# yoraish/mmd

Measured on AMD Instinct MI355X. Metric: guided trajectories/sec (H=64, 100 denoise steps), 32-robot Empty map, higher is better.
Workload: dtype f32 (f16x2 split on the fp16 MFMA pipe: every fp32 product as 3 fp16 MFMAs, fp32 accumulate)

## Files before the change

### mmd_amd/csrc/guide.hip

```cpp
#include <hip/hip_runtime.h>

#include <atomic>
#include <cmath>

#include "../../include/mmd_amd.h"
#include "../../include/mmd_amd_debug.h"
#include "bins_dev.h"
#include "common.h"
#include "guide_dev.h"

namespace mmd {

__device__ __forceinline__ float clip_scale(float gx, float gy, float gz, float gw, float max_norm) {
  const float ax = gx + 1e-6f, ay = gy + 1e-6f, az = gz + 1e-6f, aw = gw + 1e-6f;
  const float n2 = ax * ax + ay * ay + az * az + aw * aw;
  return fminf(max_norm * __builtin_amdgcn_rsqf(n2), 1.f);
}

__device__ __forceinline__ bool clip_grad(const GuideDev& g, float& gx, float& gy, float& gz, float& gw) {
  if (g.clip_rule == 0) {
    const float sc = clip_scale(gx, gy, gz, gw, g.max_norm);
    gx = sc * gx; gy = sc * gy; gz = sc * gz; gw = sc * gw;
    return sc < 1.f;
  } else if (g.clip_rule == 1) {
    const float m = g.max_value;
    const bool on = fabsf(gx) > m || fabsf(gy) > m || fabsf(gz) > m || fabsf(gw) > m;
    gx = fminf(fmaxf(gx, -m), m); gy = fminf(fmaxf(gy, -m), m); gz = fminf(fmaxf(gz, -m), m); gw = fminf(fmaxf(gw, -m), m);
    return on;
  }
  return false;
}
__device__ __forceinline__ bool clip_grad(const GuideDev& g, float& gx, float& gy) {
  float z = 0.f, w = 0.f;
  return clip_grad(g, gx, gy, z, w);
}

__device__ __forceinline__ float lane_prev(float v) {
  return __builtin_bit_cast(float, __builtin_amdgcn_update_dpp(0, __builtin_bit_cast(int, v), 0x138, 0xf, 0xf, true));
}
__device__ __forceinline__ float lane_next(float v) {
  return __builtin_bit_cast(float, __builtin_amdgcn_update_dpp(0, __builtin_bit_cast(int, v), 0x130, 0xf, 0xf, true));
}

constexpr int LDS_SLOTS_SMALL = 40;
constexpr int LDS_SLOTS_MAX = 144;

__device__ __forceinline__ float rsq_pos(float d2) { return __builtin_amdgcn_rsqf(fmaxf(d2, 1e-30f)); }

typedef float f32x2g __attribute__((ext_vector_type(2)));
struct Acc4 { f32x2g a0, a1, a2, a3; };
__device__ __forceinline__ Acc4 acc4_zero() {
  const f32x2g z = {0.f, 0.f};
  return Acc4{z, z, z, z};
}
__device__ __forceinline__ f32x2g acc4_total(const Acc4& r) {
  return f32x2g{(r.a0.x + r.a1.x) + (r.a2.x + r.a3.x), (r.a0.y + r.a1.y) + (r.a2.y + r.a3.y)};
}
__device__ __forceinline__ f32x2g cons_term(f32x2g a, f32x2g p, f32x2g q, float r2) {
  const float dx = p.x - q.x, dy = p.y - q.y;
  const float d2 = __builtin_fmaf(dx, dx, dy * dy);
  const float m = (d2 > r2) ? 0.f : rsq_pos(d2);
  return f32x2g{__builtin_fmaf(-dx, m, a.x), __builtin_fmaf(-dy, m, a.y)};
}
template <bool COMPACT> struct ConsTab;
template <> struct ConsTab<false> {
  const float4* tab;
  float r2;
  __device__ __forceinline__ f32x2g add(f32x2g a, f32x2g p, int slot, int t) const {
    const float4 c = tab[slot * H + t];
    return cons_term(a, p, f32x2g{c.x, c.y}, c.w);
  }
};
template <> struct ConsTab<true> {
  const float2* tab;
  float r2;
  __device__ __forceinline__ f32x2g add(f32x2g a, f32x2g p, int slot, int t) const {
    const float2 c = tab[slot * H + t];
    return cons_term(a, p, f32x2g{c.x, c.y}, r2);
  }
};
template <class TAB>
__device__ __forceinline__ void cons_accumulate4(Acc4& acc, const TAB& tab, int first, int n, int rel, int t, f32x2g p) {
  auto one = [&](int k, int slot) {
    if (k == 0) acc.a0 = tab.add(acc.a0, p, slot, t);
    else if (k == 1) acc.a1 = tab.add(acc.a1, p, slot, t);
    else if (k == 2) acc.a2 = tab.add(acc.a2, p, slot, t);
    else acc.a3 = tab.add(acc.a3, p, slot, t);
  };
  int i = 0;
  for (; i < n && ((rel + i) & 3); ++i) one((rel + i) & 3, first + i);
#pragma unroll 2
  for (; i + 3 < n; i += 4) {
    acc.a0 = tab.add(acc.a0, p, first + i, t);
    acc.a1 = tab.add(acc.a1, p, first + i + 1, t);
    acc.a2 = tab.add(acc.a2, p, first + i + 2, t);
    acc.a3 = tab.add(acc.a3, p, first + i + 3, t);
  }
  for (int k = 0; i < n; ++i, ++k) one(k, first + i);
}
template <class TAB>
__device__ __forceinline__ f32x2g cons_accumulate1(f32x2g a, const TAB& tab, int first, int n, int rel, int k, int t, f32x2g p) {
#pragma unroll 4
  for (int j = (k - rel) & 3; j < n; j += 4) a = tab.add(a, p, first + j, t);
  return a;
}

struct GroupMeta {
  static constexpr bool kOneGroup = false;
  int s0[2], s1[2];
  float w[2];
  int grp0, n;
  __device__ __forceinline__ void load(const GuideDev& g, int g0, int g1) {
    grp0 = g0;
    n = min(g1 - g0, 2);
#pragma unroll
    for (int k = 0; k < 2; ++k) {
      s0[k] = s1[k] = 0;
      w[k] = 0.f;
      if (k < n) {
        s0[k] = __builtin_amdgcn_readfirstlane(g.grp_slot_off[g0 + k]);
        s1[k] = __builtin_amdgcn_readfirstlane(g.grp_slot_off[g0 + k + 1]);
        w[k] = __builtin_bit_cast(float, __builtin_amdgcn_readfirstlane(__builtin_bit_cast(int, g.grp_weight[g0 + k])));
      }
    }
  }
  __device__ __forceinline__ void bounds(const GuideDev& g, int grp, int& a, int& b) const {
    const int k = grp - grp0;
    if (k == 0 && n > 0) { a = s0[0]; b = s1[0]; }
    else if (k == 1 && n > 1) { a = s0[1]; b = s1[1]; }
    else { a = __builtin_amdgcn_readfirstlane(g.grp_slot_off[grp]); b = __builtin_amdgcn_readfirstlane(g.grp_slot_off[grp + 1]); }
  }
  __device__ __forceinline__ float weight(const GuideDev& g, int grp) const {
    const int k = grp - grp0;
    return (k == 0 && n > 0) ? w[0] : (k == 1 && n > 1) ? w[1] : g.grp_weight[grp];
  }
};

template <bool DUMP = false, class GROUPSUM, class GROUPW>
__device__ __forceinline__ float4 guide_grad(const GuideDev& g, float4 xn, int t, const float4* __restrict__ grid,
                                             int grp0, int grp1, GROUPSUM group_sum, GROUPW group_weight, unsigned int* tr = nullptr) {
  unsigned int flags = 0;
  float xu[4];
  const float xv[4] = {xn.x, xn.y, xn.z, xn.w};
#pragma unroll
  for (int d = 0; d < 4; ++d) {
    float v = fminf(fmaxf(xv[d], -1.f), 1.f);
    if constexpr (DUMP) flags |= (fabsf(xv[d]) > 1.f ? 1u : 0u) << (16 + d);
    v = (v + 1.f) / 2.f;
    xu[d] = v * g.nscale[d] + g.nmin[d];
  }
  const float px = xu[0], py = xu[1], vx = xu[2], vy = xu[3];
  const bool interior = t > 0 && t < H - 1;

  int ix = (int)floorf((px - g.lo[0]) / g.dim[0] * (float)g.nx);
  int iy = (int)floorf((py - g.lo[1]) / g.dim[1] * (float)g.ny);
  ix = min(max(ix, 0), g.nx - 1);
  iy = min(max(iy, 0), g.ny - 1);
  const float4 cell0 = g.n_grids > 0 ? grid[(size_t)ix * g.ny + iy] : make_float4(1e30f, 0.f, 0.f, 0.f);

  float wsx, wsy;
  {
    const float d0 = px - g.ws_min[0], d1 = py - g.ws_min[1], d2 = g.ws_max[0] - px, d3 = g.ws_max[1] - py;
    float best = fmaxf(g.margin - d0, 0.f), gx = -1.f, gy = 0.f;
    float v = fmaxf(g.margin - d1, 0.f);
    if (v > best) { best = v; gx = 0.f; gy = -1.f; }
    v = fmaxf(g.margin - d2, 0.f);
    if (v > best) { best = v; gx = 1.f; gy = 0.f; }
    v = fmaxf(g.margin - d3, 0.f);
    if (v > best) { best = v; gx = 0.f; gy = 1.f; }
    if (!(best > 0.f)) { gx = 0.f; gy = 0.f; }
    if constexpr (DUMP) {
      const unsigned arg = gx < 0.f ? 0u : gy < 0.f ? 1u : gx > 0.f ? 2u : 3u;
      if (best > 0.f) flags |= 1u << 4 | arg << 5;
    }
    const bool clipped = clip_grad(g, gx, gy);
    if constexpr (DUMP) flags |= (clipped ? 1u : 0u) << 9;
    wsx = g.w_coll * gx; wsy = g.w_coll * gy;
  }
  float gpx, gpy, gpz, gpw;
  {
    const float npx = lane_next(px), npy = lane_next(py), nvx = lane_next(vx), nvy = lane_next(vy);
    float wpx = 0.f, wpy = 0.f, wvx = 0.f, wvy = 0.f;
    if (t < H - 1) {
      const float epx = npx - (px + g.dt * vx), epy = npy - (py + g.dt * vy);
      const float evx = nvx - vx, evy = nvy - vy;
      wpx = 2.f * (g.m1 * epx + g.m2 * evx);
      wpy = 2.f * (g.m1 * epy + g.m2 * evy);
      wvx = 2.f * (g.m2 * epx + g.m3 * evx);
      wvy = 2.f * (g.m2 * epy + g.m3 * evy);
    }
    const float lpx = lane_prev(wpx), lpy = lane_prev(wpy), lvx = lane_prev(wvx), lvy = lane_prev(wvy);
    float gx = lpx - wpx, gy = lpy - wpy;
    float gz = lvx - (g.dt * wpx + wvx), gw = lvy - (g.dt * wpy + wvy);
    const bool clipped = clip_grad(g, gx, gy, gz, gw);
    if constexpr (DUMP) flags |= (clipped ? 1u : 0u) << 10;
    gpx = g.w_smooth * gx; gpy = g.w_smooth * gy;
    gpz = g.w_smooth * gz; gpw = g.w_smooth * gw;
  }
  float cx = 0.f, cy = 0.f;
  for (int grp = grp0; grp < grp1; ++grp) {
    const f32x2g gs = group_sum(grp, f32x2g{px, py});
    float gx = gs.x, gy = gs.y;
    const bool clipped = clip_grad(g, gx, gy);
    if constexpr (DUMP) {
      const int k = grp - grp0, s0 = g.grp_slot_off[grp], s1 = g.grp_slot_off[grp + 1];
      unsigned long long mask = 0;
      unsigned int n_act = 0;
      for (int sl = s0; sl < s1; ++sl) {
        const float4 c = g.cons[(size_t)sl * H + t];
        const float dx = px - c.x, dy = py - c.y;
        const float d2 = __builtin_fmaf(dx, dx, dy * dy);
        if (!(d2 > c.w)) {
          ++n_act;
          if (sl - s0 < 64) mask |= 1ull << (sl - s0);
        }
      }
      if (k < 4) {
        tr[2 + 2 * k] = (unsigned int)mask;
        tr[3 + 2 * k] = (unsigned int)(mask >> 32);
        flags |= (clipped ? 1u : 0u) << (11 + k);
      }
      tr[10] += n_act;
    }
    const float w = group_weight(grp);
    cx += w * gx; cy += w * gy;
  }
  float ox, oy;
  {
    float best = fmaxf(g.margin - cell0.x, 0.f), gx = 0.f, gy = 0.f;
    unsigned win = 0;
    if (best > 0.f) { gx = -cell0.y; gy = -cell0.z; }
    for (int k = 1; k < g.n_grids; ++k) {
      const float4 c = grid[((size_t)k * g.nx + ix) * g.ny + iy];
      const float v = fmaxf(g.margin - c.x, 0.f);
      if (v > best) { best = v; gx = -c.y; gy = -c.z; win = (unsigned)k; }
    }
    if (g.n_xs + g.n_xb > 0) {
      float ex, ey;
      const float v = fmaxf(g.margin - extra_sdf(g.xs, g.n_xs, g.xb, g.n_xb, px, py, ex, ey), 0.f);
      if (v > best) { best = v; gx = -ex; gy = -ey; win = 7u; }
    }
    const bool clipped = clip_grad(g, gx, gy);
    if constexpr (DUMP) {
      if (best > 0.f) flags |= 1u | (win & 7u) << 1;
      flags |= (clipped ? 1u : 0u) << 8;
    }
    ox = g.w_coll * gx; oy = g.w_coll * gy;
  }
  if constexpr (DUMP) {
    tr[0] = (unsigned int)(ix * g.ny + iy);
    tr[1] = flags | (unsigned int)min(grp1 - grp0, 15) << 20;
  }
  float tx = ((ox + wsx) + gpx) + cx, ty = ((oy + wsy) + gpy) + cy;
  float tz = gpz, tw = gpw;
  if (!interior) { tx = ty = tz = tw = 0.f; }
  return make_float4(-tx, -ty, -tz, -tw);
}


template <bool COMPACT, int NT>
__device__ __forceinline__ void stage_cons(const GuideDev& g, int robot, int lds_slots, float4* lds_cons, int& lds_slot0, int& lds_n) {
  lds_slot0 = __builtin_amdgcn_readfirstlane(g.grp_slot_off[g.robot_grp_off[robot]]);
  lds_n = min(__builtin_amdgcn_readfirstlane(g.grp_slot_off[g.robot_grp_off[robot + 1]]) - lds_slot0, lds_slots);
  const float4* src = g.cons + (size_t)lds_slot0 * H;
  if constexpr (COMPACT) {
    float2* dst = reinterpret_cast<float2*>(lds_cons);
    for (int i = threadIdx.x; i < lds_n * H; i += NT) {
      const float4 c = src[i];
      dst[i] = c.z < 0.f ? make_float2(1e30f, 1e30f) : make_float2(c.x, c.y);
    }
  } else {
    for (int i = threadIdx.x; i < lds_n * H; i += NT) lds_cons[i] = src[i];
  }
}

template <bool COMPACT, class ACC>
__device__ __forceinline__ void group_slots(const GuideDev& g, const GroupMeta& gm, int grp, const float4* lds_cons, int lds_slot0, int lds_n,
                                            ACC acc) {
  int s0, s1;
  gm.bounds(g, grp, s0, s1);
  const int l0 = min(max(s0 - lds_slot0, 0), lds_n), l1 = min(max(s1 - lds_slot0, 0), lds_n);
  if (l1 > l0) {
    if constexpr (COMPACT) acc(ConsTab<true>{reinterpret_cast<const float2*>(lds_cons), g.uniform_r2}, l0, l1 - l0, lds_slot0 + l0 - s0);
    else acc(ConsTab<false>{lds_cons, 0.f}, l0, l1 - l0, lds_slot0 + l0 - s0);
  }
  const int g0 = lds_n > 0 ? max(s0, lds_slot0 + lds_n) : s0;
  if (s1 > g0) acc(ConsTab<false>{g.cons, 0.f}, g0, s1 - g0, g0 - s0);
}

__device__ __forceinline__ float4 model_update(StepDev s, float4 v, const float4* eps, size_t idx) {
  if (s.do_model)
    v = s.ddim == 2 ? ddim_update_x0(v, eps[idx], s.a_t, s.b_t, s.c1, s.c2)
        : s.ddim ? ddim_update(v, eps[idx], s.a_t, s.b_t, s.c1, s.c2) : ddpm_posterior_mean(v, eps[idx], s.a_t, s.b_t, s.c1, s.c2);
  return v;
}

template <bool DUMP, class META = GroupMeta, class GROUPSUM>
__device__ __forceinline__ void guide_iterations(const GuideDev& g, const StepDev& s, int robot, int t, size_t idx, float4& v, bool is_hard,
                                                 float4 hv, bool store, GROUPSUM group_sum) {
  const int map = g.robot_map ? g.robot_map[robot] : 0;
  const float4* grid = g.grids + (size_t)map * g.n_grids * g.nx * g.ny;
  int grp0 = 0, grp1 = 0;
  if constexpr (META::kOneGroup) {
    grp1 = 1;
  } else if (g.robot_grp_off) {
    grp0 = __builtin_amdgcn_readfirstlane(g.robot_grp_off[robot]);
    grp1 = __builtin_amdgcn_readfirstlane(g.robot_grp_off[robot + 1]);
  }
  META gm;
  if constexpr (META::kOneGroup) gm.w = group_sum.weight;
  gm.load(g, grp0, grp1);
  for (int it = 0; it < s.n_guide_steps; ++it) {
    unsigned int* tr = nullptr;
    if constexpr (DUMP) {
      tr = s.trace + ((size_t)it * s.guide_chain_stride + idx) * MMD_TRACE_WORDS;
      for (int w = 0; w < MMD_TRACE_WORDS; ++w) tr[w] = 0u;
    }
    const float4 gr = guide_grad<DUMP>(g, v, t, grid, grp0, grp1, [&](int grp, f32x2g p) { return group_sum(gm, grp, p); },
                                       [&](int grp) { return gm.weight(g, grp); }, tr);
    v.x = __builtin_fmaf(s.grad_scale, gr.x, v.x); v.y = __builtin_fmaf(s.grad_scale, gr.y, v.y);
    v.z = __builtin_fmaf(s.grad_scale, gr.z, v.z); v.w = __builtin_fmaf(s.grad_scale, gr.w, v.w);
    if (is_hard) v = hv;
    if (s.guide_chain && store) s.guide_chain[(size_t)it * s.guide_chain_stride + idx] = v;
  }
}

__device__ __forceinline__ void step_finish(const StepDev& s, float4* x, const float4* noise, float4* chain, size_t idx, int robot,
                                            int samples_per_robot, float4& v, bool is_hard, const float4& hv) {
  if (s.do_noise) v = add_step_noise(v, noise ? noise[idx] : traj_normal4(s.seed, s.robot_seeds, s.draw, s.traj_base, idx, robot, samples_per_robot), s.sigma, s.noise_std_extra);
  if (is_hard) v = hv;
  x[idx] = v;
  if (chain) chain[idx] = v;
}

template <int WPB, bool COMPACT, bool DUMP = false>
__global__ __launch_bounds__(WPB * 64) void ddpm_guide_kernel(GuideDev g, StepDev s, int lds_slots, float4* __restrict__ x,
                                                         const float4* __restrict__ eps,
                                                         const float4* __restrict__ noise, float4* __restrict__ chain,
                                                         const float4* __restrict__ hard,
                                                         int samples_per_robot) {
  extern __shared__ __attribute__((aligned(16))) float4 lds_cons[];
  const int t = threadIdx.x & 63;
  const int traj_b = s.traj0 + blockIdx.x * WPB;
  const int traj = traj_b + (threadIdx.x >> 6);
  const bool valid = traj < s.traj_end;

  int lds_slot0 = 0, lds_n = 0;
  if (s.do_guide && g.robot_grp_off) {
    const int rb0 = traj_b / samples_per_robot;
    const int rb1 = min(traj_b + WPB - 1, s.traj_end - 1) / samples_per_robot;
    if (rb0 == rb1) stage_cons<COMPACT, WPB * 64>(g, rb0, lds_slots, lds_cons, lds_slot0, lds_n);
  }
  __syncthreads();
  if (!valid) return;

  const int robot = traj / samples_per_robot;
  const size_t idx = (size_t)traj * H + t;
  float4 v = model_update(s, x[idx], eps, idx);
  float4 hv = v;
  const bool is_hard = hard_row(s.hard_rows, s.n_hard, hard, robot, t, hv);
  if constexpr (DUMP) {
    if (s.mu_out) s.mu_out[idx] = v;
  }
  if (s.do_guide)
    guide_iterations<DUMP>(g, s, robot, t, idx, v, is_hard, hv, true, [&](const GroupMeta& gm, int grp, f32x2g p) {
      Acc4 acc = acc4_zero();
      group_slots<COMPACT>(g, gm, grp, lds_cons, lds_slot0, lds_n,
                           [&](const auto& tab, int first, int n, int rel) { cons_accumulate4(acc, tab, first, n, rel, t, p); });
      return acc4_total(acc);
    });
  step_finish(s, x, noise, chain, idx, robot, samples_per_robot, v, is_hard, hv);
}

constexpr int COOP_XCH_BYTES = 2 * 4 * H * 8;
template <bool COMPACT>
__global__ __launch_bounds__(256) void ddpm_guide_coop_kernel(GuideDev g, StepDev s, int lds_slots, float4* __restrict__ x,
                                                              const float4* __restrict__ eps, const float4* __restrict__ noise,
                                                              float4* __restrict__ chain, const float4* __restrict__ hard,
                                                              int samples_per_robot) {
  extern __shared__ __attribute__((aligned(16))) float4 lds_cons[];
  const int t = threadIdx.x & 63, wave = __builtin_amdgcn_readfirstlane(threadIdx.x >> 6);
  const int traj = s.traj0 + blockIdx.x;
  const int robot = traj / samples_per_robot;
  float2* const xch = reinterpret_cast<float2*>(reinterpret_cast<char*>(lds_cons) + (size_t)lds_slots * H * (COMPACT ? 8 : 16));
  int lds_slot0 = 0, lds_n = 0;
  if (s.do_guide && g.robot_grp_off) stage_cons<COMPACT, 256>(g, robot, lds_slots, lds_cons, lds_slot0, lds_n);
  __syncthreads();
  const size_t idx = (size_t)traj * H + t;
  float4 v = model_update(s, x[idx], eps, idx);
  float4 hv = v;
  const bool is_hard = hard_row(s.hard_rows, s.n_hard, hard, robot, t, hv);
  if (s.do_guide) {
    int parity = 0;
    guide_iterations<false>(g, s, robot, t, idx, v, is_hard, hv, wave == 0, [&](const GroupMeta& gm, int grp, f32x2g p) {
      f32x2g a = {0.f, 0.f};
      group_slots<COMPACT>(g, gm, grp, lds_cons, lds_slot0, lds_n,
                           [&](const auto& tab, int first, int n, int rel) { a = cons_accumulate1(a, tab, first, n, rel, wave, t, p); });
      float2* const slot = xch + parity * 4 * H;
      slot[wave * H + t] = make_float2(a.x, a.y);
      __syncthreads();
      parity ^= 1;
      const float2 q0 = slot[t], q1 = slot[H + t], q2 = slot[2 * H + t], q3 = slot[3 * H + t];
      return acc4_total(Acc4{f32x2g{q0.x, q0.y}, f32x2g{q1.x, q1.y}, f32x2g{q2.x, q2.y}, f32x2g{q3.x, q3.y}});
    });
  }
  if (wave != 0) return;
  step_finish(s, x, noise, chain, idx, robot, samples_per_robot, v, is_hard, hv);
}


struct OneGroup {
  static constexpr bool kOneGroup = true;
  float w;
  __device__ __forceinline__ void load(const GuideDev&, int, int) {}
  __device__ __forceinline__ float weight(const GuideDev&, int) const { return w; }
};

struct BinnedSum {
  const mmd_cons_bins& b;
  int t, self;
  float r2, weight;
  __device__ __forceinline__ f32x2g operator()(const OneGroup&, int, f32x2g p) const {
    const CellList cl = own_cell_list(b, t, p.x, p.y);
    const float4 none = make_float4(0.f, 0.f, __builtin_bit_cast(float, self), 0.f);
    Acc4 acc = acc4_zero();
    const int last = max(cl.e1 - 1, 0);
    for (int e = cl.e0; __builtin_amdgcn_ballot_w64(e < cl.e1) != 0; e += 4) {
      float4 c[4];
#pragma unroll
      for (int j = 0; j < 4; ++j) {
        const float4 l = cl.ent[min(e + j, last)];
        c[j] = e + j < cl.e1 ? l : none;
      }
#pragma unroll
      for (int j = 0; j < 4; ++j) {
        const int id = __builtin_bit_cast(int, c[j].z);
        const int k = (id - (id > self ? 1 : 0)) & 3;
        f32x2g a = k == 0 ? acc.a0 : k == 1 ? acc.a1 : k == 2 ? acc.a2 : acc.a3;
        a = cons_term(a, p, f32x2g{c[j].x, c[j].y}, id != self ? r2 : -1.f);
        acc.a0 = k == 0 ? a : acc.a0;
        acc.a1 = k == 1 ? a : acc.a1;
        acc.a2 = k == 2 ? a : acc.a2;
        acc.a3 = k == 3 ? a : acc.a3;
      }
    }
    return acc4_total(acc);
  }
};

__global__ __launch_bounds__(256) void ddpm_guide_binned_kernel(GuideDev g, StepDev s, mmd_cons_bins b, float4* __restrict__ x,
                                                                const float4* __restrict__ eps, const float4* __restrict__ noise,
                                                                float4* __restrict__ chain, const float4* __restrict__ hard,
                                                                int samples_per_robot) {
  const int t = threadIdx.x & 63;
  const int traj = s.traj0 + blockIdx.x * 4 + (threadIdx.x >> 6);
  if (traj >= s.traj_end) return;
  const int robot = traj / samples_per_robot;
  const size_t idx = (size_t)traj * H + t;
  float4 v = model_update(s, x[idx], eps, idx);
  float4 hv = v;
  const bool is_hard = hard_row(s.hard_rows, s.n_hard, hard, robot, t, hv);
  if (s.do_guide)
    guide_iterations<false, OneGroup>(g, s, robot, t, idx, v, is_hard, hv, true,
                                      BinnedSum{b, t, b.robot0 + robot, b.radius * fabsf(b.radius), b.weight});
  step_finish(s, x, noise, chain, idx, robot, samples_per_robot, v, is_hard, hv);
}

__global__ void init_kernel(float4* __restrict__ x, float4* __restrict__ chain, const float4* __restrict__ hard,
                            unsigned long long hard_rows, int draw_noise, unsigned long long seed,
                            const unsigned long long* __restrict__ robot_seeds, long long traj_base, int n_traj, int samples_per_robot) {
  const size_t idx = (size_t)blockIdx.x * blockDim.x + threadIdx.x;
  if (idx >= (size_t)n_traj * H) return;
  const int t = idx % H;
  const int robot = (idx / H) / samples_per_robot;
  float4 v = draw_noise ? traj_normal4(seed, robot_seeds, 0xFFFFFFFFu, traj_base, idx, robot, samples_per_robot) : x[idx];
  float4 hv;
  if (hard_row(hard_rows, __popcll(hard_rows), hard, robot, t, hv)) v = hv;
  x[idx] = v;
  if (chain) chain[idx] = v;
}

__global__ void q_sample_kernel(float4* __restrict__ x, const float4* __restrict__ x0, const float4* __restrict__ noise,
                                float a, float b, unsigned long long seed, unsigned int draw, long long traj_base,
                                size_t n_pts) {
  const size_t idx = (size_t)blockIdx.x * blockDim.x + threadIdx.x;
  if (idx >= n_pts) return;
  const float4 z = noise ? noise[idx] : normal4(seed, draw, (unsigned long long)traj_base * H + idx);
  const float4 s = x0[idx];
  x[idx] = make_float4(a * s.x + b * z.x, a * s.y + b * z.y, a * s.z + b * z.z, a * s.w + b * z.w);
}

__global__ void cross_condition_kernel(float4* __restrict__ x1, float4* __restrict__ x2, float4* __restrict__ c1,
                                       float4* __restrict__ c2, int ind1, int ind2, float4 rel, float4 bnd,
                                       const float4* __restrict__ by_robot, int spr, int n_traj) {
  const int b = blockIdx.x * blockDim.x + threadIdx.x;
  if (b >= n_traj) return;
  if (by_robot) {
    rel = by_robot[(size_t)(b / spr) * 2];
    bnd = by_robot[(size_t)(b / spr) * 2 + 1];
  }
  const float4 v2 = x2[(size_t)b * H + ind2];
  float4 v1;
  v1.x = fminf(v2.x + rel.x, bnd.x); v1.y = fminf(v2.y + rel.y, bnd.y);
  v1.z = fminf(v2.z + rel.z, bnd.z); v1.w = fminf(v2.w + rel.w, bnd.w);
  x1[(size_t)b * H + ind1] = v1;
  float4 w;
  w.x = fmaxf(v1.x - rel.x, -bnd.x); w.y = fmaxf(v1.y - rel.y, -bnd.y);
  w.z = fmaxf(v1.z - rel.z, -bnd.z); w.w = fmaxf(v1.w - rel.w, -bnd.w);
  x2[(size_t)b * H + ind2] = w;
  if (c1) c1[(size_t)b * H + ind1] = v1;
  if (c2) c2[(size_t)b * H + ind2] = w;
}

int fill_guide(const mmd_guide_desc* d, GuideDev& g) {
  MMD_REQUIRE(d->n_grids == 0 || (d->sdf_grids_dev && d->grid_nx >= 1 && d->grid_ny >= 1), "guide: SDF grid missing");
  if (d->cons_bins) {
    MMD_REQUIRE(!d->cons_ell_dev, "guide: cons_bins together with an ELL table (cons_ell_dev) is not supported");
    if (int rc = check_cons_bins(d->cons_bins)) return rc;
  }
  for (int k = 0; k < 4; ++k) { g.nmin[k] = d->norm_min[k]; g.nscale[k] = d->norm_max[k] - d->norm_min[k]; }
  for (int k = 0; k < 2; ++k) {
    g.lo[k] = d->limits_lo[k];
    g.dim[k] = fabsf(d->limits_hi[k] - d->limits_lo[k]);
    g.ws_min[k] = d->ws_min[k]; g.ws_max[k] = d->ws_max[k];
  }
  g.nx = d->grid_nx; g.ny = d->grid_ny; g.n_grids = d->n_grids;
  g.grids = reinterpret_cast<const float4*>(d->sdf_grids_dev);
  g.robot_map = d->robot_map_dev;
  g.margin = d->margin; g.dt = d->dt; g.w_coll = d->weight_collision; g.w_smooth = d->weight_smoothness;
  g.max_norm = d->max_grad_norm;
  MMD_REQUIRE(d->clip_grad_rule >= 0 && d->clip_grad_rule <= 2, "guide: clip_grad_rule must be 0 (norm), 1 (value) or 2 (off)");
  g.clip_rule = d->clip_grad_rule;
  g.max_value = d->max_grad_value;
  const double dt = d->dt, qc = 1.0 / ((double)d->sigma_gp * d->sigma_gp);
  g.m1 = (float)(12.0 / (dt * dt * dt) * qc);
  g.m2 = (float)(-6.0 / (dt * dt) * qc);
  g.m3 = (float)(4.0 / dt * qc);
  g.max_slots = d->max_slots_per_robot > 0 ? d->max_slots_per_robot : LDS_SLOTS_SMALL;
  g.uniform_r2 = d->cons_uniform_radius > 0.f ? d->cons_uniform_radius * fabsf(d->cons_uniform_radius) : 0.f;
  g.xs = reinterpret_cast<const float4*>(d->extra_spheres_dev); g.n_xs = d->extra_spheres_dev ? d->n_extra_spheres : 0;
  g.xb = reinterpret_cast<const float4*>(d->extra_boxes_dev); g.n_xb = d->extra_boxes_dev ? d->n_extra_boxes : 0;
  g.cons = reinterpret_cast<const float4*>(d->cons_ell_dev);
  g.grp_slot_off = d->grp_slot_off_dev; g.grp_weight = d->grp_weight_dev; g.robot_grp_off = d->robot_grp_off_dev;
  if (!g.cons || !g.grp_slot_off || !g.grp_weight) g.robot_grp_off = nullptr;
  return 0;
}

constexpr int kCoopMaxTrajDefault = 512;

int launch_step(const GuideDev& g, StepDev s, float* x, const float* eps, const float* noise, float* chain,
                const float* hard, int traj0, int n_traj, int spr, hipStream_t st, const mmd_cons_bins* bins) {
  s.traj0 = traj0;
  s.traj_end = traj0 + n_traj;
  if (bins && s.do_guide) {
    hipLaunchKernelGGL(ddpm_guide_binned_kernel, dim3((n_traj + 3) / 4), dim3(256), 0, st, g, s, *bins, (float4*)x, (const float4*)eps,
                       (const float4*)noise, (float4*)chain, (const float4*)hard, spr);
    return 0;
  }
  const bool guided = s.do_guide && g.robot_grp_off;
  const bool compact = guided && g.uniform_r2 > 0.f;
  const int bytes_per_slot = H * (compact ? 8 : 16);
  const int small = LDS_SLOTS_SMALL * (compact ? 2 : 1), big = LDS_SLOTS_MAX * (compact ? 2 : 1);
  auto launch = [&](auto kern, int grid, int block, size_t lds_bytes, int slots) {
    hipLaunchKernelGGL(kern, dim3(grid), dim3(block), lds_bytes, st, g, s, slots, (float4*)x, (const float4*)eps, (const float4*)noise,
                       (float4*)chain, (const float4*)hard, spr);
  };
  if (s.trace) {
    launch(ddpm_guide_kernel<4, false, true>, (n_traj + 3) / 4, 256, 0, 0);
  } else if (guided && n_traj <= (s.coop_max > 0 ? s.coop_max : s.coop_max < 0 ? 0 : kCoopMaxTrajDefault)) {
    const int fit = 60 * 1024 / bytes_per_slot;
    const int slots = g.max_slots < fit ? g.max_slots : fit;
    launch(compact ? ddpm_guide_coop_kernel<true> : ddpm_guide_coop_kernel<false>, n_traj, 256,
           (size_t)slots * bytes_per_slot + COOP_XCH_BYTES, slots);
  } else if (guided && g.max_slots > small && spr % 8 == 0 && traj0 % 8 == 0) {
    const int slots = g.max_slots < big ? g.max_slots : big;
    static std::atomic<unsigned long long> attr_devices{0};
    int dev = 0;
    (void)hipGetDevice(&dev);
    const unsigned long long bit = 1ull << (dev & 63);
    if (!(attr_devices.load(std::memory_order_acquire) & bit)) {
      (void)hipFuncSetAttribute(reinterpret_cast<const void*>(&ddpm_guide_kernel<8, false>),
                                hipFuncAttributeMaxDynamicSharedMemorySize, LDS_SLOTS_MAX * H * 16);
      (void)hipFuncSetAttribute(reinterpret_cast<const void*>(&ddpm_guide_kernel<8, true>),
                                hipFuncAttributeMaxDynamicSharedMemorySize, LDS_SLOTS_MAX * H * 16);
      attr_devices.fetch_or(bit, std::memory_order_release);
    }
    launch(compact ? ddpm_guide_kernel<8, true> : ddpm_guide_kernel<8, false>, (n_traj + 7) / 8, 512, (size_t)slots * bytes_per_slot, slots);
  } else {
    const int slots = guided ? small : 0;
    launch(compact ? ddpm_guide_kernel<4, true> : ddpm_guide_kernel<4, false>, (n_traj + 3) / 4, 256, (size_t)slots * bytes_per_slot, slots);
  }
  return 0;
}

void launch_cross(float* x1, float* x2, float* c1, float* c2, int ind1, int ind2, const float* rel, const float* bnd,
                  const float* by_robot, int spr, int n_traj, hipStream_t st) {
  hipLaunchKernelGGL(cross_condition_kernel, dim3((n_traj + 255) / 256), dim3(256), 0, st, (float4*)x1, (float4*)x2,
                     (float4*)c1, (float4*)c2, ind1, ind2, make_float4(rel[0], rel[1], rel[2], rel[3]),
                     make_float4(bnd[0], bnd[1], bnd[2], bnd[3]), (const float4*)by_robot, spr > 0 ? spr : 1, n_traj);
}

int launch_init(float* x, float* chain, const float* hard, unsigned long long hard_rows, int draw, unsigned long long seed,
                const unsigned long long* robot_seeds, long long traj_base, int n_traj, int spr, hipStream_t st) {
  const size_t n = (size_t)n_traj * H;
  hipLaunchKernelGGL(init_kernel, dim3((unsigned)((n + 255) / 256)), dim3(256), 0, st, (float4*)x, (float4*)chain,
                     (const float4*)hard, hard_rows, draw, seed, robot_seeds, traj_base, n_traj, spr);
  return 0;
}

}

using namespace mmd;

extern "C" {

int mmd_guide_steps(const mmd_guide_desc* d, float* x_dev, const float* hard_dev, uint64_t hard_rows, int n_robots,
                    int samples_per_robot, int n_steps, float* chain_dev, void* stream) {
  MMD_REQUIRE(d && x_dev && hard_dev, "mmd_guide_steps: NULL argument");
  GuideDev g{};
  if (int rc = fill_guide(d, g)) return rc;
  StepDev s{};
  s.do_guide = 1; s.n_guide_steps = n_steps; s.hard_rows = hard_rows; s.n_hard = __builtin_popcountll(hard_rows); s.grad_scale = 1.f;
  s.guide_chain = reinterpret_cast<float4*>(chain_dev);
  s.guide_chain_stride = (long long)n_robots * samples_per_robot * H;
  launch_step(g, s, x_dev, nullptr, nullptr, nullptr, hard_dev, 0, n_robots * samples_per_robot, samples_per_robot,
              (hipStream_t)stream, d->cons_bins);
  MMD_HIP_CHECK(hipGetLastError());
  return 0;
}

int mmd_q_sample(float* x_dev, const float* x_start_dev, const float* noise_dev, float a, float b, uint64_t seed,
                 uint32_t draw_index, int64_t traj_index_base, int n_traj, void* stream) {
  MMD_REQUIRE(x_dev && x_start_dev && n_traj >= 1, "mmd_q_sample: bad arguments");
  const size_t n = (size_t)n_traj * H;
  hipLaunchKernelGGL(q_sample_kernel, dim3((unsigned)((n + 255) / 256)), dim3(256), 0, (hipStream_t)stream,
                     (float4*)x_dev, (const float4*)x_start_dev, (const float4*)noise_dev, a, b,
                     (unsigned long long)seed, draw_index, (long long)traj_index_base, n);
  MMD_HIP_CHECK(hipGetLastError());
  return 0;
}

int mmd_cross_condition(float* x1_dev, float* x2_dev, int ind1, int ind2, const float* rel, const float* boundary,
                        int n_traj, void* stream) {
  MMD_REQUIRE(x1_dev && x2_dev && rel && boundary, "mmd_cross_condition: NULL argument");
  MMD_REQUIRE(ind1 >= 0 && ind1 < H && ind2 >= 0 && ind2 < H, "row index out of range");
  launch_cross(x1_dev, x2_dev, nullptr, nullptr, ind1, ind2, rel, boundary, nullptr, 1, n_traj, (hipStream_t)stream);
  MMD_HIP_CHECK(hipGetLastError());
  return 0;
}

}
```

Measured before the change: 95170.

## Pad staged constraint table and software-pipeline LDS loads; hoist map-free obstacle term

```diff
diff --git a/mmd_amd/csrc/guide.hip b/mmd_amd/csrc/guide.hip
--- a/mmd_amd/csrc/guide.hip
+++ b/mmd_amd/csrc/guide.hip
@@ -7,6 +7,7 @@
 #include "../../include/mmd_amd_debug.h"
 #include "bins_dev.h"
 #include "common.h"
+#include "cons_table_dev.h"
 #include "guide_dev.h"
 
 namespace mmd {
@@ -44,6 +45,7 @@
 
 constexpr int LDS_SLOTS_SMALL = 40;
 constexpr int LDS_SLOTS_MAX = 144;
+static_assert(LDS_SLOTS_SMALL % 8 == 0 && LDS_SLOTS_MAX % 8 == 0, "a staged table is padded to a multiple of 8 slots inside these (stage_cons)");
 
 __device__ __forceinline__ float rsq_pos(float d2) { return __builtin_amdgcn_rsqf(fmaxf(d2, 1e-30f)); }
 
@@ -64,20 +66,20 @@
 }
 template <bool COMPACT> struct ConsTab;
 template <> struct ConsTab<false> {
+  typedef float4 entry;
   const float4* tab;
   float r2;
-  __device__ __forceinline__ f32x2g add(f32x2g a, f32x2g p, int slot, int t) const {
-    const float4 c = tab[slot * H + t];
-    return cons_term(a, p, f32x2g{c.x, c.y}, c.w);
-  }
+  static __device__ __forceinline__ entry none() { return empty_word(); }
+  __device__ __forceinline__ f32x2g term(f32x2g a, f32x2g p, entry c) const { return cons_term(a, p, f32x2g{c.x, c.y}, c.w); }
+  __device__ __forceinline__ f32x2g add(f32x2g a, f32x2g p, int slot, int t) const { return term(a, p, tab[slot * H + t]); }
 };
 template <> struct ConsTab<true> {
+  typedef float2 entry;
   const float2* tab;
   float r2;
-  __device__ __forceinline__ f32x2g add(f32x2g a, f32x2g p, int slot, int t) const {
-    const float2 c = tab[slot * H + t];
-    return cons_term(a, p, f32x2g{c.x, c.y}, r2);
-  }
+  static __device__ __forceinline__ entry none() { return make_float2(1e30f, 1e30f); }
+  __device__ __forceinline__ f32x2g term(f32x2g a, f32x2g p, entry c) const { return cons_term(a, p, f32x2g{c.x, c.y}, r2); }
+  __device__ __forceinline__ f32x2g add(f32x2g a, f32x2g p, int slot, int t) const { return term(a, p, tab[slot * H + t]); }
 };
 template <class TAB>
 __device__ __forceinline__ void cons_accumulate4(Acc4& acc, const TAB& tab, int first, int n, int rel, int t, f32x2g p) {
@@ -136,8 +138,59 @@
   }
 };
 
+__device__ __forceinline__ float4 no_cell() { return make_float4(1e30f, 0.f, 0.f, 0.f); }
+
+template <bool DUMP>
+__device__ __forceinline__ f32x2g map_term(const GuideDev& g, const float4* __restrict__ grid, int ix, int iy, float4 cell0, float px, float py,
+                                           unsigned int& flags) {
+  float best = fmaxf(g.margin - cell0.x, 0.f), gx = 0.f, gy = 0.f;
+  unsigned win = 0;
+  if (best > 0.f) { gx = -cell0.y; gy = -cell0.z; }
+  for (int k = 1; k < g.n_grids; ++k) {
+    const float4 c = grid[((size_t)k * g.nx + ix) * g.ny + iy];
+    const float v = fmaxf(g.margin - c.x, 0.f);
+    if (v > best) { best = v; gx = -c.y; gy = -c.z; win = (unsigned)k; }
+  }
+  if (g.n_xs + g.n_xb > 0) {
+    float ex, ey;
+    const float v = fmaxf(g.margin - extra_sdf(g.xs, g.n_xs, g.xb, g.n_xb, px, py, ex, ey), 0.f);
+    if (v > best) { best = v; gx = -ex; gy = -ey; win = 7u; }
+  }
+  const bool clipped = clip_grad(g, gx, gy);
+  if constexpr (DUMP) {
+    if (best > 0.f) flags |= 1u | (win & 7u) << 1;
+    flags |= (clipped ? 1u : 0u) << 8;
+  }
+  return f32x2g{g.w_coll * gx, g.w_coll * gy};
+}
+
+struct MapFree {
+  bool on;
+  f32x2g o;
+};
+template <bool DUMP>
+__device__ __forceinline__ MapFree map_free_term(const GuideDev& g) {
+  MapFree m{!DUMP && g.n_grids == 0 && g.n_xs + g.n_xb == 0, f32x2g{0.f, 0.f}};
+  if (m.on) {
+    GuideDev e = g;
+    e.n_grids = e.n_xs = e.n_xb = 0;
+    unsigned int flags = 0;
+    const f32x2g o = map_term<false>(e, nullptr, 0, 0, no_cell(), 0.f, 0.f, flags);
+    m.o.x = __builtin_bit_cast(float, __builtin_amdgcn_readfirstlane(__builtin_bit_cast(int, o.x)));
+    m.o.y = __builtin_bit_cast(float, __builtin_amdgcn_readfirstlane(__builtin_bit_cast(int, o.y)));
+  }
+  return m;
+}
+
+struct OneGroup {
+  static constexpr bool kOneGroup = true;
+  float w;
+  __device__ __forceinline__ void load(const GuideDev&, int, int) {}
+  __device__ __forceinline__ float weight(const GuideDev&, int) const { return w; }
+};
+
 template <bool DUMP = false, class GROUPSUM, class GROUPW>
-__device__ __forceinline__ float4 guide_grad(const GuideDev& g, float4 xn, int t, const float4* __restrict__ grid,
+__device__ __forceinline__ float4 guide_grad(const GuideDev& g, float4 xn, int t, const float4* __restrict__ grid, const MapFree& mf,
                                              int grp0, int grp1, GROUPSUM group_sum, GROUPW group_weight, unsigned int* tr = nullptr) {
   unsigned int flags = 0;
   float xu[4];
@@ -152,11 +205,16 @@
   const float px = xu[0], py = xu[1], vx = xu[2], vy = xu[3];
   const bool interior = t > 0 && t < H - 1;
 
-  int ix = (int)floorf((px - g.lo[0]) / g.dim[0] * (float)g.nx);
-  int iy = (int)floorf((py - g.lo[1]) / g.dim[1] * (float)g.ny);
-  ix = min(max(ix, 0), g.nx - 1);
-  iy = min(max(iy, 0), g.ny - 1);
-  const float4 cell0 = g.n_grids > 0 ? grid[(size_t)ix * g.ny + iy] : make_float4(1e30f, 0.f, 0.f, 0.f);
+  int ix, iy;
+  float4 cell0;
+  if (!mf.on) {
+    cell0 = no_cell();
+    ix = (int)floorf((px - g.lo[0]) / g.dim[0] * (float)g.nx);
+    iy = (int)floorf((py - g.lo[1]) / g.dim[1] * (float)g.ny);
+    ix = min(max(ix, 0), g.nx - 1);
+    iy = min(max(iy, 0), g.ny - 1);
+    if (g.n_grids > 0) cell0 = grid[(size_t)ix * g.ny + iy];
+  }
 
   float wsx, wsy;
   {
@@ -225,28 +283,9 @@
     const float w = group_weight(grp);
     cx += w * gx; cy += w * gy;
   }
-  float ox, oy;
-  {
-    float best = fmaxf(g.margin - cell0.x, 0.f), gx = 0.f, gy = 0.f;
-    unsigned win = 0;
-    if (best > 0.f) { gx = -cell0.y; gy = -cell0.z; }
-    for (int k = 1; k < g.n_grids; ++k) {
-      const float4 c = grid[((size_t)k * g.nx + ix) * g.ny + iy];
-      const float v = fmaxf(g.margin - c.x, 0.f);
-      if (v > best) { best = v; gx = -c.y; gy = -c.z; win = (unsigned)k; }
-    }
-    if (g.n_xs + g.n_xb > 0) {
-      float ex, ey;
-      const float v = fmaxf(g.margin - extra_sdf(g.xs, g.n_xs, g.xb, g.n_xb, px, py, ex, ey), 0.f);
-      if (v > best) { best = v; gx = -ex; gy = -ey; win = 7u; }
-    }
-    const bool clipped = clip_grad(g, gx, gy);
-    if constexpr (DUMP) {
-      if (best > 0.f) flags |= 1u | (win & 7u) << 1;
-      flags |= (clipped ? 1u : 0u) << 8;
-    }
-    ox = g.w_coll * gx; oy = g.w_coll * gy;
-  }
+  f32x2g o = mf.o;
+  if (!mf.on) o = map_term<DUMP>(g, grid, ix, iy, cell0, px, py, flags);
+  const float ox = o.x, oy = o.y;
   if constexpr (DUMP) {
     tr[0] = (unsigned int)(ix * g.ny + iy);
     tr[1] = flags | (unsigned int)min(grp1 - grp0, 15) << 20;
@@ -258,20 +297,22 @@
 }
 
 
-template <bool COMPACT, int NT>
+template <bool COMPACT, int NT, bool PAD>
 __device__ __forceinline__ void stage_cons(const GuideDev& g, int robot, int lds_slots, float4* lds_cons, int& lds_slot0, int& lds_n) {
   lds_slot0 = __builtin_amdgcn_readfirstlane(g.grp_slot_off[g.robot_grp_off[robot]]);
   lds_n = min(__builtin_amdgcn_readfirstlane(g.grp_slot_off[g.robot_grp_off[robot + 1]]) - lds_slot0, lds_slots);
   const float4* src = g.cons + (size_t)lds_slot0 * H;
+  typename ConsTab<COMPACT>::entry* dst = reinterpret_cast<typename ConsTab<COMPACT>::entry*>(lds_cons);
   if constexpr (COMPACT) {
-    float2* dst = reinterpret_cast<float2*>(lds_cons);
     for (int i = threadIdx.x; i < lds_n * H; i += NT) {
       const float4 c = src[i];
-      dst[i] = c.z < 0.f ? make_float2(1e30f, 1e30f) : make_float2(c.x, c.y);
+      dst[i] = c.z < 0.f ? ConsTab<true>::none() : make_float2(c.x, c.y);
     }
   } else {
     for (int i = threadIdx.x; i < lds_n * H; i += NT) lds_cons[i] = src[i];
   }
+  if constexpr (PAD)
+    for (int i = lds_n * H + threadIdx.x; i < ((lds_n + 7) & ~7) * H; i += NT) dst[i] = ConsTab<COMPACT>::none();
 }
 
 template <bool COMPACT, class ACC>
@@ -287,6 +328,49 @@
   const int g0 = lds_n > 0 ? max(s0, lds_slot0 + lds_n) : s0;
   if (s1 > g0) acc(ConsTab<false>{g.cons, 0.f}, g0, s1 - g0, g0 - s0);
 }
+
+template <bool COMPACT>
+struct PaddedSum {
+  typedef typename ConsTab<COMPACT>::entry entry;
+  ConsTab<COMPACT> tab;
+  int n8, t;
+  float weight;
+  entry first[8];
+  __device__ __forceinline__ void load(entry (&c)[8], int slot) const {
+#pragma unroll
+    for (int j = 0; j < 8; ++j) c[j] = tab.tab[(slot + j) * H + t];
+    __builtin_amdgcn_sched_barrier(0);
+  }
+  __device__ __forceinline__ void apply(Acc4& acc, const entry (&c)[8], f32x2g p) const {
+#pragma unroll
+    for (int j = 0; j < 8; j += 4) {
+      acc.a0 = tab.term(acc.a0, p, c[j]);
+      acc.a1 = tab.term(acc.a1, p, c[j + 1]);
+      acc.a2 = tab.term(acc.a2, p, c[j + 2]);
+      acc.a3 = tab.term(acc.a3, p, c[j + 3]);
+    }
+  }
+  __device__ __forceinline__ void hold_first() {
+    load(first, 0);
+    __builtin_amdgcn_s_waitcnt(0xc07f);
+  }
+  __device__ __forceinline__ f32x2g operator()(const OneGroup&, int, f32x2g p) const {
+    Acc4 acc = acc4_zero();
+    entry b[8], c[8];
+    const int last = n8 - 8;
+    load(b, min(8, last));
+    apply(acc, first, p);
+    int i = 8;
+    for (; i + 8 <= last; i += 16) {
+      load(c, i + 8);
+      apply(acc, b, p);
+      load(b, min(i + 16, last));
+      apply(acc, c, p);
+    }
+    if (i <= last) apply(acc, b, p);
+    return acc4_total(acc);
+  }
+};
 
 __device__ __forceinline__ float4 model_update(StepDev s, float4 v, const float4* eps, size_t idx) {
   if (s.do_model)
@@ -310,13 +394,14 @@
   META gm;
   if constexpr (META::kOneGroup) gm.w = group_sum.weight;
   gm.load(g, grp0, grp1);
+  const MapFree mf = map_free_term<DUMP>(g);
   for (int it = 0; it < s.n_guide_steps; ++it) {
     unsigned int* tr = nullptr;
     if constexpr (DUMP) {
       tr = s.trace + ((size_t)it * s.guide_chain_stride + idx) * MMD_TRACE_WORDS;
       for (int w = 0; w < MMD_TRACE_WORDS; ++w) tr[w] = 0u;
     }
-    const float4 gr = guide_grad<DUMP>(g, v, t, grid, grp0, grp1, [&](int grp, f32x2g p) { return group_sum(gm, grp, p); },
+    const float4 gr = guide_grad<DUMP>(g, v, t, grid, mf, grp0, grp1, [&](int grp, f32x2g p) { return group_sum(gm, grp, p); },
                                        [&](int grp) { return gm.weight(g, grp); }, tr);
     v.x = __builtin_fmaf(s.grad_scale, gr.x, v.x); v.y = __builtin_fmaf(s.grad_scale, gr.y, v.y);
     v.z = __builtin_fmaf(s.grad_scale, gr.z, v.z); v.w = __builtin_fmaf(s.grad_scale, gr.w, v.w);
@@ -349,7 +434,7 @@
   if (s.do_guide && g.robot_grp_off) {
     const int rb0 = traj_b / samples_per_robot;
     const int rb1 = min(traj_b + WPB - 1, s.traj_end - 1) / samples_per_robot;
-    if (rb0 == rb1) stage_cons<COMPACT, WPB * 64>(g, rb0, lds_slots, lds_cons, lds_slot0, lds_n);
+    if (rb0 == rb1) stage_cons<COMPACT, WPB * 64, true>(g, rb0, lds_slots, lds_cons, lds_slot0, lds_n);
   }
   __syncthreads();
   if (!valid) return;
@@ -362,7 +447,20 @@
   if constexpr (DUMP) {
     if (s.mu_out) s.mu_out[idx] = v;
   }
-  if (s.do_guide)
+  bool padded = false;
+  if constexpr (!DUMP) {
+    if (s.do_guide && lds_n > 0) {
+      const int g0 = __builtin_amdgcn_readfirstlane(g.robot_grp_off[robot]), g1 = __builtin_amdgcn_readfirstlane(g.robot_grp_off[robot + 1]);
+      padded = g1 - g0 == 1 && __builtin_amdgcn_readfirstlane(g.grp_slot_off[g1]) - lds_slot0 == lds_n;
+      if (padded) {
+        const float w = __builtin_bit_cast(float, __builtin_amdgcn_readfirstlane(__builtin_bit_cast(int, g.grp_weight[g0])));
+        PaddedSum<COMPACT> sum{{reinterpret_cast<const typename ConsTab<COMPACT>::entry*>(lds_cons), g.uniform_r2}, (lds_n + 7) & ~7, t, w};
+        sum.hold_first();
+        guide_iterations<false, OneGroup>(g, s, robot, t, idx, v, is_hard, hv, true, sum);
+      }
+    }
+  }
+  if (s.do_guide && !padded)
     guide_iterations<DUMP>(g, s, robot, t, idx, v, is_hard, hv, true, [&](const GroupMeta& gm, int grp, f32x2g p) {
       Acc4 acc = acc4_zero();
       group_slots<COMPACT>(g, gm, grp, lds_cons, lds_slot0, lds_n,
@@ -384,7 +482,7 @@
   const int robot = traj / samples_per_robot;
   float2* const xch = reinterpret_cast<float2*>(reinterpret_cast<char*>(lds_cons) + (size_t)lds_slots * H * (COMPACT ? 8 : 16));
   int lds_slot0 = 0, lds_n = 0;
-  if (s.do_guide && g.robot_grp_off) stage_cons<COMPACT, 256>(g, robot, lds_slots, lds_cons, lds_slot0, lds_n);
+  if (s.do_guide && g.robot_grp_off) stage_cons<COMPACT, 256, false>(g, robot, lds_slots, lds_cons, lds_slot0, lds_n);
   __syncthreads();
   const size_t idx = (size_t)traj * H + t;
   float4 v = model_update(s, x[idx], eps, idx);
@@ -408,13 +506,6 @@
   step_finish(s, x, noise, chain, idx, robot, samples_per_robot, v, is_hard, hv);
 }
 
-
-struct OneGroup {
-  static constexpr bool kOneGroup = true;
-  float w;
-  __device__ __forceinline__ void load(const GuideDev&, int, int) {}
-  __device__ __forceinline__ float weight(const GuideDev&, int) const { return w; }
-};
 
 struct BinnedSum {
   const mmd_cons_bins& b;
@@ -585,7 +676,8 @@
                                 hipFuncAttributeMaxDynamicSharedMemorySize, LDS_SLOTS_MAX * H * 16);
       attr_devices.fetch_or(bit, std::memory_order_release);
     }
-    launch(compact ? ddpm_guide_kernel<8, true> : ddpm_guide_kernel<8, false>, (n_traj + 7) / 8, 512, (size_t)slots * bytes_per_slot, slots);
+    launch(compact ? ddpm_guide_kernel<8, true> : ddpm_guide_kernel<8, false>, (n_traj + 7) / 8, 512,
+           (size_t)((slots + 7) & ~7) * bytes_per_slot, slots);
   } else {
     const int slots = guided ? small : 0;
     launch(compact ? ddpm_guide_kernel<4, true> : ddpm_guide_kernel<4, false>, (n_traj + 3) / 4, 256, (size_t)slots * bytes_per_slot, slots);
```

Result: faster. 96940, median of 6 (+1.9%).
